# bcgsc/abyss

Measured on NVIDIA H100. Metric: k-mers/sec (Bloom insert + unitig extend), higher is better.
Workload: dtype u8

## Files before the change

abyss_b200/csrc/abb_api.cu:

```cuda
#include "abb_common.h"
#include "abb_insert.cuh"
#include "abb_shard.cuh"
#include <dlfcn.h>
#include <nccl.h>
#include <cub/device/device_scan.cuh>
#include <algorithm>
#include <cstdlib>
#include <cstring>
#include <new>
#include <vector>

namespace abb {

static thread_local char g_err[512] = "";

void set_error(const char* fmt, ...)
{
	va_list ap;
	va_start(ap, fmt);
	vsnprintf(g_err, sizeof g_err, fmt, ap);
	va_end(ap);
}

constexpr uint64_t kDefaultWindow = 1ULL << 17;
constexpr uint64_t kChunkSlots = 1ULL << 27;

static uint64_t next_pow2(uint64_t x)
{
	uint64_t p = 1;
	while (p < x)
		p <<= 1;
	return p;
}

int select_device(int device)
{
	int n = 0;
	cudaError_t e = cudaGetDeviceCount(&n);
	if (e != cudaSuccess || n <= 0) {
		set_error("no usable CUDA device (%s); libabyssb200 has no CPU fallback",
		          e == cudaSuccess ? "device count is 0" : cudaGetErrorString(e));
		return ABB_ENODEV;
	}
	if (device < 0 || device >= n) {
		set_error("device %d out of range (0..%d)", device, n - 1);
		return ABB_EINVAL;
	}
	ABB_CUDA(cudaSetDevice(device));
	return ABB_OK;
}

static FilterView view_of(const abb_filter* f)
{
	FilterView v;
	v.data = f->d_data.p;
	v.level_stride = f->level_stride();
	v.levels = f->levels;
	return v;
}

constexpr unsigned kMapLog2 = 25;
constexpr unsigned kShardMapLog2 = 27;

static uint64_t map_entries_for(uint64_t filter_size, unsigned lg)
{
	const uint64_t fit = std::max<uint64_t>(next_pow2(filter_size), 1024);
	return std::min<uint64_t>(1ULL << lg, fit);
}

static unsigned age_windows_for(uint64_t window)
{
	return (unsigned)std::min<uint64_t>(kMaxAgeWindows, ((1ULL << kPrioBits) - 2) / window - 1);
}

static int ensure_workspace(abb_filter* f, uint64_t window, unsigned lg)
{
	const uint64_t want_entries = map_entries_for(f->size, lg);
	if (f->d_carry.p && f->ws_window == window && f->ws_H == f->H && f->map_entries == want_entries)
		return ABB_OK;
	f->ws_window = 0;
	f->d_map[0] = f->d_map[1] = f->d_map[2] = nullptr;
	f->maps.reset();
	f->d_tags2[0].reset();
	f->d_tags2[1].reset();
	f->d_carry.reset();
	f->d_slotbits.reset();
	const size_t map_words = std::max<size_t>(want_entries / 4, 256) / sizeof(unsigned);
	f->tag_slots = next_pow2(8ULL * kCarryLanes * f->H);
	ABB_CHECK(f->maps.alloc(3 * map_words));
	ABB_CUDA(cudaMemsetAsync(f->maps.p, 0, 3 * map_words * sizeof(unsigned), f->stream));
	for (auto& tags : f->d_tags2) {
		ABB_CHECK(tags.alloc(f->tag_slots));
		ABB_CUDA(cudaMemsetAsync(tags.p, 0, f->tag_slots * sizeof(unsigned long long), f->stream));
	}
	ABB_CHECK(f->d_carry.alloc(3 * (window + kCarryLanes)));
	f->slotbit_words = ((uint64_t)age_windows_for(window) + 3) * window / 32 + 64;
	ABB_CHECK(f->d_slotbits.alloc(f->slotbit_words));
	ABB_CUDA(cudaMemsetAsync(f->d_slotbits.p, 0, f->slotbit_words * sizeof(unsigned), f->stream));
	for (int i = 0; i < 3; ++i)
		f->d_map[i] = f->maps.p + i * map_words;
	f->map_entries = want_entries;
	f->ws_window = window;
	f->ws_H = f->H;
	return ABB_OK;
}

#define ABB_DISPATCH_H(H, ...)            \
	do {                                  \
		if ((H) <= 4) {                   \
			constexpr int MAXH = 4;       \
			__VA_ARGS__;                  \
		} else if ((H) <= 8) {            \
			constexpr int MAXH = 8;       \
			__VA_ARGS__;                  \
		} else {                          \
			constexpr int MAXH = 32;      \
			__VA_ARGS__;                  \
		}                                 \
	} while (0)

static void set_l2_policy(abb_filter* f, bool on, int n_maps = 3)
{
	cudaStreamAttrValue attr;
	memset(&attr, 0, sizeof attr);
	if (on) {
		int max_persist = 0, max_window = 0;
		cudaDeviceGetAttribute(&max_persist, cudaDevAttrMaxPersistingL2CacheSize, f->device);
		cudaDeviceGetAttribute(&max_window, cudaDevAttrMaxAccessPolicyWindowSize, f->device);
		const size_t bytes = (size_t)n_maps * std::max<size_t>(f->map_entries / 4, 256);
		if (max_persist <= 0 || max_window <= 0)
			return;
		cudaDeviceSetLimit(cudaLimitPersistingL2CacheSize, std::min<size_t>(bytes, (size_t)max_persist));
		attr.accessPolicyWindow.base_ptr = f->d_map[0];
		attr.accessPolicyWindow.num_bytes = std::min<size_t>(bytes, (size_t)max_window);
		attr.accessPolicyWindow.hitRatio = std::min(1.0f, (float)max_persist / (float)bytes);
		attr.accessPolicyWindow.hitProp = cudaAccessPropertyPersisting;
		attr.accessPolicyWindow.missProp = cudaAccessPropertyStreaming;
	} else {
		attr.accessPolicyWindow.num_bytes = 0;
		attr.accessPolicyWindow.hitProp = cudaAccessPropertyNormal;
		attr.accessPolicyWindow.missProp = cudaAccessPropertyNormal;
	}
	cudaStreamSetAttribute(f->stream, cudaStreamAttributeAccessPolicyWindow, &attr);
	if (!on) {
		cudaCtxResetPersistingL2Cache();
		cudaDeviceSetLimit(cudaLimitPersistingL2CacheSize, 0);
	}
	cudaGetLastError();
}

struct PolicyHold {
	abb_filter* f;
	bool took;
	PolicyHold(abb_filter* f_, int n_maps) : f(f_), took(!f_->l2_policy_held && f_->d_map[0] != nullptr)
	{
		if (took) {
			set_l2_policy(f, true, n_maps);
			f->l2_policy_held = true;
		}
	}
	~PolicyHold()
	{
		if (took) {
			set_l2_policy(f, false);
			f->l2_policy_held = false;
		}
	}
	PolicyHold(const PolicyHold&) = delete;
	PolicyHold& operator=(const PolicyHold&) = delete;
};

template <int KIND, bool LITERAL, int MAXH>
static int launch_windows(const InsertArgs& args, int device, cudaStream_t st)
{
	static int grid_cache[64] = { 0 };
	int& grid = grid_cache[device & 63];
	if (grid == 0) {
		int per_sm = 0, sms = 0;
		ABB_CUDA(cudaOccupancyMaxActiveBlocksPerMultiprocessor(&per_sm, k_insert_windows<KIND, LITERAL, MAXH>, 256, 0));
		ABB_CUDA(cudaDeviceGetAttribute(&sms, cudaDevAttrMultiProcessorCount, device));
		grid = std::max(1, per_sm) * sms;
	}
	void* params[] = { (void*)&args };
	ABB_CUDA(cudaLaunchCooperativeKernel((void*)k_insert_windows<KIND, LITERAL, MAXH>, dim3((unsigned)grid), dim3(256), params, 0, st));
	return ABB_OK;
}

static int fold_profile(abb_filter* f)
{
	if (!f->profile || !f->prof_used)
		return ABB_OK;
	ABB_CUDA(cudaStreamSynchronize(f->stream));
	for (size_t i = 0; i + 1 < f->prof_used; i += 2) {
		float ms = 0;
		cudaEventElapsedTime(&ms, f->prof_ev[i], f->prof_ev[i + 1]);
		f->st.ms_commit += ms;
		f->st.commit_launches += 1;
	}
	f->st.commit_slots += f->prof_slots;
	f->prof_used = 0;
	f->prof_slots = 0;
	return ABB_OK;
}

template <bool LITERAL>
static int ordered_insert(abb_filter* f, const uint64_t* d_hashes, const uint8_t* d_valid, uint64_t n_slots)
{
	if (n_slots == 0)
		return ABB_OK;
	if (f->kind == ABB_BIT) {
		ABB_DISPATCH_H(f->H, (k_bits_insert<LITERAL, MAXH><<<blocks_for(n_slots, 256), 256, 0, f->stream>>>(
		                         d_hashes, d_valid, n_slots, f->cfg, f->d_data.p)));
		f->st.launches += 1;
		ABB_CUDA(cudaGetLastError());
		return ABB_OK;
	}
	ABB_CHECK(ensure_workspace(f, f->window, kMapLog2));
	cudaStream_t st = f->stream;
	const uint64_t W = f->window;
	const uint64_t n_windows = (n_slots + W - 1) / W;
	ABB_REQUIRE(n_windows < (1ULL << 31), "too many windows in one call");
	const uint64_t cap = W + kCarryLanes;
	InsertArgs a;
	a.hashes = d_hashes;
	a.valid = d_valid;
	a.n_slots = n_slots;
	a.window = (unsigned)W;
	a.w_begin = 0;
	a.n_windows = (unsigned)n_windows;
	a.cfg = f->cfg;
	for (int i = 0; i < 3; ++i) {
		a.map[i].w = f->d_map[i];
		a.map[i].mask = f->map_entries - 1;
	}
	for (int i = 0; i < 2; ++i) {
		a.tags[i] = f->d_tags2[i].p;
		a.carry[i] = f->d_carry.p + (uint64_t)i * cap;
	}
	a.tag_cap = (unsigned)f->tag_slots;
	a.f = view_of(f);
	a.age_off = (unsigned)(age_windows_for(W) * W);
	a.drain_age = a.age_off / 3 * 2;
	a.ctl = f->d_ctl.p;
	a.stats = f->d_stats.p;
	uint64_t* sorted = f->d_carry.p + 2 * cap;
	ABB_CUDA(cudaMemsetAsync(f->d_ctl.p, 0, sizeof(InsertCtl), st));
	ABB_CUDA(cudaMemsetAsync(f->d_map[0], 0, 3 * std::max<size_t>(f->map_entries / 4, 256), st));
	for (int i = 0; i < 2; ++i)
		ABB_CUDA(cudaMemsetAsync(f->d_tags2[i].p, 0, f->tag_slots * sizeof(unsigned long long), st));
	const bool counting = f->kind == ABB_COUNTING;
	PolicyHold policy(f, 3);
	while (a.w_begin < a.n_windows) {
		const bool timed = f->profile && f->prof_used + 2 <= f->prof_ev.size();
		if (timed)
			cudaEventRecord(f->prof_ev[f->prof_used++], st);
		ABB_DISPATCH_H(f->H, {
			if (counting)
				ABB_CHECK((launch_windows<0, LITERAL, MAXH>(a, f->device, st)));
			else
				ABB_CHECK((launch_windows<1, LITERAL, MAXH>(a, f->device, st)));
		});
		if (timed)
			cudaEventRecord(f->prof_ev[f->prof_used++], st);
		InsertCtl h;
		ABB_CUDA(cudaMemcpyAsync(&h, f->d_ctl.p, sizeof h, cudaMemcpyDeviceToHost, st));
		ABB_CUDA(cudaStreamSynchronize(st));
		ABB_REQUIRE(h.resume > a.w_begin && h.resume <= a.n_windows, "insert kernel made no progress (window %u of %u)", h.resume, a.n_windows);
		if (timed)
			f->prof_slots += std::min<uint64_t>(n_slots, (uint64_t)h.resume * W) - (uint64_t)a.w_begin * W;
		const int which = 1 - (int)((h.resume - 1) & 1);
		const uint64_t w0 = (uint64_t)(h.resume - 1) * W;
		const uint64_t lo_slot = w0 > (uint64_t)a.age_off + W ? w0 - a.age_off - W : 0;
		ABB_DISPATCH_H(f->H, {
			if (counting)
				k_drain<0, LITERAL, MAXH><<<1, kDrainThreads, 0, st>>>(d_hashes, f->cfg, a.f, a.carry[which], a.ctl, which, 0, 1, f->d_slotbits.p, lo_slot,
				                                                      sorted, f->d_stats.p);
			else
				k_drain<1, LITERAL, MAXH><<<1, kDrainThreads, 0, st>>>(d_hashes, f->cfg, a.f, a.carry[which], a.ctl, which, 0, 1, f->d_slotbits.p, lo_slot,
				                                                      sorted, f->d_stats.p);
		});
		f->st.launches += 2;
		f->st.windows += h.resume - a.w_begin;
		a.w_begin = h.resume;
	}
	ABB_CUDA(cudaGetLastError());
	return fold_profile(f);
}

__global__ void k_chunk_bounds(const uint64_t* __restrict__ slot_offs, uint64_t n_reads, uint64_t cap,
                               uint64_t* __restrict__ bounds, unsigned max_chunks, unsigned* __restrict__ n_chunks)
{
	uint64_t r = 0;
	unsigned c = 0;
	bounds[0] = 0;
	while (r < n_reads && c + 1 < max_chunks) {
		const uint64_t limit = slot_offs[r] + cap;
		uint64_t lo = r + 1, hi = n_reads;
		while (lo < hi) {
			uint64_t mid = lo + (hi - lo + 1) / 2;
			if (slot_offs[mid] <= limit)
				lo = mid;
			else
				hi = mid - 1;
		}
		r = lo;
		bounds[++c] = r;
	}
	if (r < n_reads)
		bounds[++c] = n_reads;
	*n_chunks = c;
}

__global__ void __launch_bounds__(256)
k_count_valid(const uint8_t* __restrict__ valid, uint64_t n, unsigned long long* __restrict__ out)
{
	unsigned long long c = 0;
	for (uint64_t i = (uint64_t)blockIdx.x * blockDim.x + threadIdx.x; i < n; i += (uint64_t)gridDim.x * blockDim.x)
// ... 186 lines not shown
		f->st.ms_insert += ms;
		f->st.slots += slots;
	}
	unsigned long long nk = 0;
	ABB_CUDA(cudaMemcpyAsync(&nk, f->d_stats.p + kStatInsertKmers, sizeof nk, cudaMemcpyDeviceToHost, f->stream));
	ABB_CUDA(cudaStreamSynchronize(f->stream));
	f->st.kmers += nk;
	if (n_kmers_out)
		*n_kmers_out = nk;
	return ABB_OK;
}

struct NcclApi {
	void* h = nullptr;
	ncclResult_t (*GetUniqueId)(ncclUniqueId*) = nullptr;
	ncclResult_t (*CommInitRank)(ncclComm_t*, int, ncclUniqueId, int) = nullptr;
	ncclResult_t (*CommDestroy)(ncclComm_t) = nullptr;
	ncclResult_t (*AllReduce)(const void*, void*, size_t, ncclDataType_t, ncclRedOp_t, ncclComm_t, cudaStream_t) = nullptr;
	ncclResult_t (*AllGather)(const void*, void*, size_t, ncclDataType_t, ncclComm_t, cudaStream_t) = nullptr;
	ncclResult_t (*Send)(const void*, size_t, ncclDataType_t, int, ncclComm_t, cudaStream_t) = nullptr;
	ncclResult_t (*Recv)(void*, size_t, ncclDataType_t, int, ncclComm_t, cudaStream_t) = nullptr;
	ncclResult_t (*GroupStart)() = nullptr;
	ncclResult_t (*GroupEnd)() = nullptr;
	const char* (*GetErrorString)(ncclResult_t) = nullptr;
};
static NcclApi g_nccl;

static int load_nccl()
{
	if (g_nccl.h)
		return ABB_OK;
	const char* names[] = { getenv("ABB_NCCL_LIB"), "libnccl.so.2", "libnccl.so" };
	void* h = nullptr;
	for (const char* n : names)
		if (n && *n && (h = dlopen(n, RTLD_NOW | RTLD_GLOBAL)))
			break;
	if (!h) {
		set_error("cannot load NCCL (libnccl.so.2): %s", dlerror());
		return ABB_ENODEV;
	}
#define ABB_NCCL_SYM(field, name)                                        \
	do {                                                                 \
		*(void**)(&g_nccl.field) = dlsym(h, name);                       \
		if (!g_nccl.field) {                                             \
			set_error("NCCL library lacks %s", name);                    \
			return ABB_ENODEV;                                           \
		}                                                                \
	} while (0)
	ABB_NCCL_SYM(GetUniqueId, "ncclGetUniqueId");
	ABB_NCCL_SYM(CommInitRank, "ncclCommInitRank");
	ABB_NCCL_SYM(CommDestroy, "ncclCommDestroy");
	ABB_NCCL_SYM(AllReduce, "ncclAllReduce");
	ABB_NCCL_SYM(AllGather, "ncclAllGather");
	ABB_NCCL_SYM(Send, "ncclSend");
	ABB_NCCL_SYM(Recv, "ncclRecv");
	ABB_NCCL_SYM(GroupStart, "ncclGroupStart");
	ABB_NCCL_SYM(GroupEnd, "ncclGroupEnd");
	ABB_NCCL_SYM(GetErrorString, "ncclGetErrorString");
#undef ABB_NCCL_SYM
	g_nccl.h = h;
	return ABB_OK;
}

#define ABB_NCCL(call)                                                                                   \
	do {                                                                                                 \
		ncclResult_t r__ = (call);                                                                       \
		if (r__ != ncclSuccess) {                                                                        \
			abb::set_error("%s:%d: %s failed: %s", __FILE__, __LINE__, #call, g_nccl.GetErrorString(r__)); \
			return ABB_ECUDA;                                                                            \
		}                                                                                                \
	} while (0)

}

struct abb_comm {
	ncclComm_t comm = nullptr;
	int rank = 0, world = 1, device = 0;
};

namespace abb {

static uint64_t shard_chunk(uint64_t size, unsigned world) { return ((size + world - 1) / world + 15) & ~15ULL; }

static uint64_t sharded_window(const abb_filter* f, unsigned world)
{
	const uint64_t w = 2 * f->window * world;
	return std::min<uint64_t>(std::max<uint64_t>(w, 32), 1ULL << 21);
}

static int sharded_ordered_insert(abb_filter* f, abb_comm* c, const uint64_t* d_h0, const uint8_t* d_valid, uint64_t n_slots)
{
	if (n_slots == 0)
		return ABB_OK;
	const uint64_t W = sharded_window(f, (unsigned)c->world);
	ABB_CHECK(ensure_workspace(f, W, kShardMapLog2));
	const unsigned max_lanes = (unsigned)std::min<uint64_t>((uint64_t)kCarryLanes * (unsigned)c->world, W / 2 + kCarryLanes);
	ABB_CHECK(f->sh_buf.reserve(2 * (W + (uint64_t)max_lanes) + 64));
	cudaStream_t st = f->stream;
	const uint64_t n_windows = (n_slots + W - 1) / W;
	const unsigned age_off = (unsigned)(age_windows_for(W) * W);
	const unsigned drain_age = age_off / 3 * 2;
	const uint64_t cap = 3 * (W + kCarryLanes) / 2;
	uint64_t* carry[2] = { f->d_carry.p, f->d_carry.p + cap };
	ShardCtl* ctl = f->d_shard_ctl.p;
	const size_t map_bytes = std::max<size_t>(f->map_entries / 4, 256);
	ConflictMap maps[2] = { { f->d_map[0], f->map_entries - 1 }, { f->d_map[1], f->map_entries - 1 } };
	const uint64_t chunk = shard_chunk(f->size, (unsigned)c->world);
	Shard sh;
	sh.lo = std::min<uint64_t>(f->size, (uint64_t)c->rank * chunk);
	sh.hi = std::min<uint64_t>(f->size, sh.lo + chunk);
	{
		ShardCtl init;
		init.n_pending = 0;
		init.n_out = 0;
		init.lo_pending = ~0ULL;
		ABB_CUDA(cudaMemcpyAsync(ctl, &init, sizeof init, cudaMemcpyHostToDevice, st));
	}
	ABB_CUDA(cudaMemsetAsync(f->d_map[0], 0, 3 * map_bytes, st));
	unsigned n_in = 0;
	uint64_t oldest = 0;
	int in = 0, p = 0;
	uint8_t* buf = f->sh_buf.p;
	auto step = [&](uint64_t w0, unsigned n, uint64_t w1, unsigned n_next) -> int {
		const unsigned lanes_c = std::min<unsigned>(n_in, max_lanes);
		uint64_t tslots = 4096;
		while (tslots < 8ULL * lanes_c * f->H / (unsigned)c->world + 4096 && tslots < f->tag_slots)
			tslots <<= 1;
		const TagTable tab = { f->d_tags2[0].p, std::min<uint64_t>(tslots, f->tag_slots) - 1 };
		if (lanes_c)
			ABB_CUDA(cudaMemsetAsync(tab.e, 0, (tab.mask + 1) * sizeof(unsigned long long), st));
		const unsigned lanes = lanes_c + n;
		const uint64_t lo_slot = w0 > (uint64_t)age_off + W ? w0 - age_off - W : 0;
		uint8_t* pm = buf;
		uint8_t* ok = buf + lanes;
		const bool timed = f->profile && n && (f->st.windows % f->prof_stride) == 0 && f->prof_used + 2 <= f->prof_ev.size();
		ABB_DISPATCH_H(f->H, {
			if (lanes_c)
				k_sh_mark_carry<false, MAXH><<<blocks_for(lanes_c, 256), 256, 0, st>>>(d_h0, carry[in], lanes_c, w0, f->cfg, tab, age_off, maps[p], sh);
			if (timed)
				cudaEventRecord(f->prof_ev[f->prof_used++], st);
			k_sh_gather<false, MAXH><<<blocks_for((uint64_t)lanes_c + std::max(n, n_next), 256), 256, 0, st>>>(
			    d_h0, d_valid, w0, n, w1, n_next, f->cfg, maps[p], maps[1 - p], tab, f->d_data.p, age_off, carry[in], lanes_c, sh, pm, ok);
		});
		if (lanes) {
			ABB_NCCL(g_nccl.AllReduce(buf, buf, 2 * (size_t)lanes, ncclUint8, ncclMin, c->comm, st));
			ABB_DISPATCH_H(f->H, (k_sh_apply<false, MAXH><<<blocks_for((uint64_t)n_in + n, 256), 256, 0, st>>>(
			                         d_h0, d_valid, w0, n, f->cfg, tab, f->d_data.p, carry[in], n_in, lanes_c, sh, pm, ok, f->d_slotbits.p, lo_slot, ctl,
			                         f->d_stats.p)));
			if (timed) {
				cudaEventRecord(f->prof_ev[f->prof_used++], st);
				f->prof_slots += n;
			}
			k_sh_compact<<<1, kDrainThreads, 0, st>>>(f->d_slotbits.p, lo_slot, w0 + std::max<uint64_t>(n, 1), carry[1 - in], ctl, &ctl->n_out);
			unsigned h_n = 0;
			ABB_CUDA(cudaMemcpyAsync(&h_n, &ctl->n_out, sizeof h_n, cudaMemcpyDeviceToHost, st));
			ABB_CUDA(cudaMemcpyAsync(&oldest, carry[1 - in], sizeof oldest, cudaMemcpyDeviceToHost, st));
			ABB_CUDA(cudaStreamSynchronize(st));
			n_in = h_n;
			in = 1 - in;
			f->st.launches += 4;
		} else {
			if (timed)
				f->prof_used--;
			f->st.launches += 1;
		}
		return ABB_OK;
	};
	auto drain = [&](uint64_t w0, unsigned until) -> int {
		while (n_in > until) {
			ABB_CHECK(step(w0, 0, w0, 0));
			f->sh_drains += 1;
		}
		return ABB_OK;
	};
	f->prof_stride = f->prof_ev.empty() ? 1 : std::max<uint64_t>(1, (2 * n_windows + f->prof_ev.size() - 1) / f->prof_ev.size());
	PolicyHold policy(f, 2);
	ABB_CHECK(step(0, 0, 0, (unsigned)std::min<uint64_t>(W, n_slots)));
	p = 1 - p;
// ... 4 lines not shown
		const unsigned n_next = w + 1 < n_windows ? (unsigned)std::min<uint64_t>(W, n_slots - w1) : 0u;
		if (n_in > max_lanes)
			ABB_CHECK(drain(w0, max_lanes / 2));
		if (n_in && w0 - oldest > drain_age)
			ABB_CHECK(drain(w0, 0));
		ABB_CHECK(step(w0, n, w1, n_next));
		ABB_CUDA(cudaMemsetAsync(maps[p].w, 0, map_bytes, st));
		p = 1 - p;
		f->st.windows += 1;
	}
	ABB_CHECK(drain(n_slots, 0));
	ABB_CUDA(cudaGetLastError());
	return fold_profile(f);
}

}

using namespace abb;

extern "C" {

int abb_version(void) { return ABB_VERSION; }
const char* abb_last_error(void) { return g_err; }

int abb_device_count(void)
{
	int n = 0;
	cudaError_t e = cudaGetDeviceCount(&n);
	if (e != cudaSuccess) {
		set_error("cudaGetDeviceCount: %s", cudaGetErrorString(e));
		return ABB_ENODEV;
	}
	return n;
}

static int alloc_filter(std::unique_ptr<abb_filter> f, abb_filter** out);

int abb_filter_create(abb_filter** out, int kind, uint64_t size, unsigned num_hashes, unsigned k, unsigned arg,
                      const char* mask, int device)
{
	ABB_REQUIRE(out != nullptr, "abb_filter_create: out is NULL");
	*out = nullptr;
	ABB_REQUIRE(kind != ABB_KONNECTOR, "Konnector filters are created with abb_konnector_create");
	ABB_REQUIRE(kind == ABB_COUNTING || kind == ABB_BIT || kind == ABB_CASCADING, "unknown filter kind %d", kind);
	ABB_REQUIRE(num_hashes >= 1 && num_hashes <= kMaxHashes, "number of hash functions must be in 1..%u (MAX_HASHES)", kMaxHashes);
	ABB_REQUIRE(k >= 1 && k <= kMaxK, "k-mer size must be in 1..%u (MAX_KMER)", kMaxK);
	if (kind == ABB_COUNTING) {
		if (size % 8)
			size += 8 - size % 8;
	} else {
		ABB_REQUIRE(size % 8 == 0, "ERROR: Filter Size \"%llu\" is not a multiple of 8.", (unsigned long long)size);
	}
	ABB_REQUIRE(size >= 8, "filter size must be at least 8");
	ABB_REQUIRE(size < (1ULL << kPosBits), "filter size %llu exceeds the supported maximum 2^%u", (unsigned long long)size, kPosBits);
	unsigned levels = 1;
	if (kind == ABB_CASCADING) {
		ABB_REQUIRE(arg >= 1 && arg <= 255, "cascading filter needs 1..255 levels");
		levels = arg;
	}
	std::string m = mask ? mask : "";
	if (!m.empty()) {
		ABB_REQUIRE(m.size() == k, "spaced seed must be exactly k=%u characters long", k);
		for (char c : m)
			ABB_REQUIRE(c == '0' || c == '1', "spaced seed must contain only '0' and '1'");
		if (m.find('0') == std::string::npos)
			m.clear();
	}
	ABB_CHECK(select_device(device));

	std::unique_ptr<abb_filter> f(new (std::nothrow) abb_filter());
	if (!f) {
		set_error("out of host memory");
		return ABB_ENOMEM;
	}
	f->device = device;
	f->kind = kind;
	f->size = size;
	f->bytes_per_level = kind == ABB_COUNTING ? size : size / 8;
	f->H = num_hashes;
	f->k = k;
	f->threshold = kind == ABB_COUNTING ? arg : 0;
	f->levels = levels;
	f->mask = m;
	f->window = kDefaultWindow;
	f->cfg.H = num_hashes;
	f->cfg.k = k;
	f->cfg.mod = make_fastmod(size);
	for (unsigned i = 0; i < kMaxHashes; ++i)
		f->cfg.mult[i] = (uint64_t)i ^ ((uint64_t)k * kMultiSeed);
	return alloc_filter(std::move(f), out);
}

static int alloc_filter(std::unique_ptr<abb_filter> f, abb_filter** out)
{
	const unsigned k = f->k, levels = f->levels;
	ABB_CUDA(cudaStreamCreateWithFlags(f->stream.out(), cudaStreamNonBlocking));
	ABB_CUDA(cudaEventCreate(f->ev0.out()));
	ABB_CUDA(cudaEventCreate(f->ev1.out()));
	ABB_CHECK(f->d_data.alloc(f->level_stride() * levels + 4096));
	ABB_CUDA(cudaMemsetAsync(f->d_data.p, 0, f->level_stride() * levels, f->stream));
	ABB_CHECK(f->d_ctl.alloc(1));
	ABB_CUDA(cudaMemsetAsync(f->d_ctl.p, 0, sizeof(InsertCtl), f->stream));
	ABB_CHECK(f->d_shard_ctl.alloc(1));
	ABB_CHECK(f->d_stats.alloc(kStatWords));
	ABB_CUDA(cudaMemsetAsync(f->d_stats.p, 0, kStatWords * sizeof(unsigned long long), f->stream));
	if (!f->mask.empty()) {
		std::vector<uint8_t> care(k);
		for (unsigned i = 0; i < k; ++i)
			care[i] = f->mask[i] == '1';
		ABB_CHECK(f->d_care.alloc(k));
		ABB_CUDA(cudaMemcpyAsync(f->d_care.p, care.data(), k, cudaMemcpyHostToDevice, f->stream));
	}
	ABB_CUDA(cudaStreamSynchronize(f->stream));
	return hand_over(f, out);
}

int abb_konnector_create(abb_filter** out, uint64_t full_bits, unsigned k, unsigned levels, uint64_t hash_seed, uint64_t start_bit,
                         uint64_t end_bit, int device)
{
	ABB_REQUIRE(out != nullptr, "abb_konnector_create: out is NULL");
	*out = nullptr;
	ABB_REQUIRE(k >= 1 && k <= kMaxK, "k-mer size must be in 1..%u (MAX_KMER)", kMaxK);
	ABB_REQUIRE(full_bits >= 2, "a Konnector filter needs at least 2 bits");
	ABB_REQUIRE(start_bit <= end_bit && end_bit < full_bits, "window [%llu, %llu] is not inside a filter of %llu bits",
	            (unsigned long long)start_bit, (unsigned long long)end_bit, (unsigned long long)full_bits);
	ABB_REQUIRE(levels >= 1 && levels <= 255, "a Konnector filter needs 1..255 levels");
	ABB_CHECK(select_device(device));
	std::unique_ptr<abb_filter> f(new (std::nothrow) abb_filter());
	if (!f) {
		set_error("out of host memory");
		return ABB_ENOMEM;
	}
	f->device = device;
	f->kind = ABB_KONNECTOR;
	f->size = end_bit - start_bit + 1;
	f->bytes_per_level = (f->size + 7) / 8;
	f->H = 1;
	f->k = k;
	f->levels = levels;
	f->kon_full = full_bits;
	f->kon_start = start_bit;
	f->kon_seed = hash_seed;
	return alloc_filter(std::move(f), out);
}

int abb_filter_destroy(abb_filter* f)
{
	if (!f)
		return ABB_OK;
	cudaSetDevice(f->device);
	cudaStreamSynchronize(f->stream);
	if (f->copy_stream)
		cudaStreamSynchronize(f->copy_stream);
	delete f;
	return ABB_OK;
}

unsigned abb_filter_kmer_size(const abb_filter* f) { return f ? f->k : 0; }
unsigned abb_filter_hash_num(const abb_filter* f) { return f ? f->H : 0; }
uint64_t abb_filter_size(const abb_filter* f) { return f ? f->size : 0; }
uint64_t abb_filter_size_in_bytes(const abb_filter* f) { return f ? f->bytes_per_level : 0; }
unsigned abb_filter_threshold(const abb_filter* f) { return f ? f->threshold : 0; }
unsigned abb_filter_levels(const abb_filter* f) { return f ? f->levels : 0; }

int abb_filter_set_threshold(abb_filter* f, unsigned threshold)
{
	ABB_REQUIRE(f, "NULL filter");
	if (f->kind != ABB_COUNTING) {
		set_error("threshold only applies to counting filters");
		return ABB_ESTATE;
	}
	f->threshold = threshold;
	return ABB_OK;
}

int abb_filter_set_profiling(abb_filter* f, int on)
{
	ABB_REQUIRE(f, "NULL filter");
	ABB_CUDA(cudaSetDevice(f->device));
	f->profile = on != 0;
	if (f->profile && f->prof_ev.empty()) {
		std::vector<Event> ev(2048);
		for (auto& e : ev)
			ABB_CUDA(cudaEventCreate(e.out()));
		f->prof_ev = std::move(ev);
	}
	return ABB_OK;
}

int abb_filter_set_window(abb_filter* f, uint64_t window_slots)
{
	ABB_REQUIRE(f, "NULL filter");
	if (window_slots == 0)
		window_slots = kDefaultWindow;
	ABB_REQUIRE(window_slots >= 32 && window_slots <= (1ULL << 20) - 64, "window must be in [32, 2^20 - 64]");
	ABB_CUDA(cudaSetDevice(f->device));
	ABB_CUDA(cudaStreamSynchronize(f->stream));
	f->window = window_slots;
	return ABB_OK;
}

int abb_insert_reads_dev(abb_filter* f, const char* d_bases, const uint64_t* d_offsets, uint64_t n_reads,
                         uint64_t n_bases, uint64_t* n_kmers_out)
{
	(void)n_bases;
	ABB_REQUIRE(f, "NULL filter");
	ABB_REQUIRE(n_reads == 0 || (d_bases && d_offsets), "NULL read buffers");
	ABB_CUDA(cudaSetDevice(f->device));
	if (f->kind == ABB_KONNECTOR)
		return kon_insert_reads_dev(f, (const uint8_t*)d_bases, d_offsets, n_reads, n_kmers_out);
	return insert_reads_dev(f, (const uint8_t*)d_bases, d_offsets, n_reads, n_kmers_out);
}

int abb_insert_reads(abb_filter* f, const char* bases, const uint64_t* offsets, uint64_t n_reads, uint64_t* n_kmers_out)
{
	ABB_REQUIRE(f, "NULL filter");
	if (n_kmers_out)
		*n_kmers_out = 0;
	if (n_reads == 0)
		return ABB_OK;
	ABB_CHECK(check_read_batch(bases, offsets, n_reads));
	const uint64_t n_bases = offsets[n_reads];
	ABB_CUDA(cudaSetDevice(f->device));
	constexpr uint64_t kPiece = 256ULL << 20;
	const bool in_pieces = f->kind != ABB_KONNECTOR && n_bases > kPiece;
	ABB_CHECK(stage_read_batch(in_pieces ? nullptr : bases, offsets, n_reads, f->bases, f->offs, f->stream));
	f->resident_reads = n_reads;
	if (f->kind == ABB_KONNECTOR)
		return kon_insert_reads_dev(f, f->bases.p, f->offs.p, n_reads, n_kmers_out);
	if (!in_pieces)
		return insert_reads_dev(f, f->bases.p, f->offs.p, n_reads, n_kmers_out);
	if (!f->copy_stream)
		ABB_CUDA(cudaStreamCreateWithFlags(f->copy_stream.out(), cudaStreamNonBlocking));
	if (f->kind != ABB_BIT)
		ABB_CHECK(ensure_workspace(f, f->window, kMapLog2));
	PolicyHold policy(f, 3);
	PendingCopy pc;
	pc.h_offs = offsets;
	pc.piece = kPiece;
	pc.n_pieces = (size_t)((n_bases + kPiece - 1) / kPiece);
	while (f->copy_ev.size() < pc.n_pieces) {
		Event ev;
		ABB_CUDA(cudaEventCreateWithFlags(ev.out(), cudaEventDisableTiming));
		f->copy_ev.push_back(std::move(ev));
	}
	ABB_CUDA(cudaEventRecord(f->ev0, f->stream));
	ABB_CUDA(cudaStreamWaitEvent(f->copy_stream, f->ev0, 0));
	for (size_t i = 0; i < pc.n_pieces; ++i) {
		const uint64_t b0 = (uint64_t)i * kPiece, b1 = std::min<uint64_t>(n_bases, b0 + kPiece);
		ABB_CUDA(cudaMemcpyAsync(f->bases.p + b0, bases + b0, b1 - b0, cudaMemcpyHostToDevice, f->copy_stream));
		ABB_CUDA(cudaEventRecord(f->copy_ev[i], f->copy_stream));
	}
	const int rc = insert_reads_dev(f, f->bases.p, f->offs.p, n_reads, n_kmers_out, nullptr, &pc);
	ABB_CUDA(cudaStreamSynchronize(f->copy_stream));
	return rc;
}

static bool shard_policy(int world)
{
	static int min_world = -1;
	if (min_world < 0) {
		const char* e = getenv("ABB_SHARD_MIN_WORLD");
		min_world = e ? std::max(2, atoi(e)) : 4;
	}
	return world > 1 && world >= min_world;
}

int abb_insert_reads_sharded(abb_filter* f, abb_comm* c, const char* bases, const uint64_t* offsets, uint64_t n_reads, int finalize,
                             uint64_t* n_kmers_out)
{
	ABB_REQUIRE(f && c, "NULL argument");
	ABB_REQUIRE_NTHASH(f);
	if (!shard_policy(c->world)) {
		ABB_REQUIRE(f->kind == ABB_COUNTING, "the sharded insert is implemented for counting filters");
		ABB_REQUIRE(f->device == c->device, "filter and communicator live on different devices");
		f->replicated_insert = true;
		(void)finalize;
		return abb_insert_reads(f, bases, offsets, n_reads, n_kmers_out);
	}
	if (n_kmers_out)
		*n_kmers_out = 0;
	ABB_CHECK(check_read_batch(bases, offsets, n_reads));
	ABB_CUDA(cudaSetDevice(f->device));
	ABB_CHECK(stage_read_batch(bases, offsets, n_reads, f->bases, f->offs, f->stream));
	f->resident_reads = n_reads;
	return abb_insert_reads_sharded_dev(f, c, (const char*)f->bases.p, f->offs.p, n_reads, finalize, n_kmers_out);
}

int abb_filter_resident_reads(abb_filter* f, const char** d_bases, const uint64_t** d_offsets, uint64_t* n_reads)
{
	ABB_REQUIRE(f && d_bases && d_offsets && n_reads, "NULL argument");
	*d_bases = (const char*)f->bases.p;
	*d_offsets = f->offs.p;
	*n_reads = f->resident_reads;
	return ABB_OK;
}

int abb_insert_hashes(abb_filter* f, const uint64_t* hashes, uint64_t n)
{
	ABB_REQUIRE(f, "NULL filter");
	ABB_REQUIRE_NTHASH(f);
	if (n == 0)
		return ABB_OK;
	ABB_REQUIRE(hashes, "NULL hashes");
	ABB_CUDA(cudaSetDevice(f->device));
	ABB_CHECK(f->lit.reserve(n * f->H));
	ABB_CUDA(cudaMemcpyAsync(f->lit.p, hashes, n * f->H * sizeof(uint64_t), cudaMemcpyHostToDevice, f->stream));
	ABB_CHECK(ordered_insert<true>(f, f->lit.p, nullptr, n));
	ABB_CUDA(cudaStreamSynchronize(f->stream));
	f->st.kmers += n;
	return ABB_OK;
}

int abb_hash_reads_dev(abb_filter* f, const char* d_bases, const uint64_t* d_offsets, uint64_t n_reads, uint64_t* d_h0,
                       uint8_t* d_valid, uint64_t capacity, uint64_t* n_slots_out)
{
	ABB_REQUIRE(f, "NULL filter");
	ABB_REQUIRE_NTHASH(f);
// ... 457 lines not shown
```

abyss_b200/csrc/abb_insert.cuh:

```cuda
#pragma once
#include "abb_common.h"
#include "abb_device.cuh"
#include "abb_graph.cuh"
#include <cooperative_groups.h>
#include <cuda/barrier>
#include <cuda_runtime.h>

namespace abb {
namespace cg = cooperative_groups;

constexpr unsigned kPrioBits = 28;
constexpr unsigned kMaxAgeWindows = 48;
constexpr unsigned kCarryLanes = 1u << 16;
constexpr unsigned kPosBits = 36;
constexpr uint64_t kPrioMask = (1ULL << kPrioBits) - 1;

struct TagTable {
	unsigned long long* e;
	uint64_t mask;
};

ABB_D uint64_t tag_pack(uint64_t pos, uint64_t prio) { return ((pos + 1) << kPrioBits) | prio; }
ABB_D uint64_t tag_home(uint64_t pos, const TagTable& t)
{
// ... 246 lines not shown
static __global__ void __launch_bounds__(kHashWarps * 32)
k_hash_segments(const uint8_t* __restrict__ bases, const uint64_t* __restrict__ seg_beg, const unsigned* __restrict__ seg_len,
                const uint64_t* __restrict__ seg_slot, uint64_t n_segs, unsigned k, uint64_t* __restrict__ h0_out,
                uint8_t* __restrict__ valid_out)
{
	__shared__ uint64_t sP[kHashWarps][kRing];
	__shared__ uint64_t sQ[kHashWarps][kRing];
	__shared__ unsigned sB[kHashWarps][kRing];
	const int warp = threadIdx.x >> 5, lane = threadIdx.x & 31;
	for (uint64_t r = (uint64_t)blockIdx.x * kHashWarps + warp; r < n_segs; r += (uint64_t)gridDim.x * kHashWarps) {
		const unsigned L = seg_len[r];
		if (L < k)
			continue;
		hash_one_read(bases, seg_beg[r], L, seg_slot[r], k, sP[warp], sQ[warp], sB[warp], lane, h0_out, valid_out);
	}
}

static __global__ void __launch_bounds__(kHashWarps * 32)
k_hash_reads_masked(const uint8_t* __restrict__ bases, const uint64_t* __restrict__ offs,
                    const uint64_t* __restrict__ slot_offs, uint64_t slot_base, uint64_t n_reads, unsigned k,
                    const uint8_t* __restrict__ care, uint64_t* __restrict__ h0_out, uint8_t* __restrict__ valid_out)
{
	const int warp = threadIdx.x >> 5, lane = threadIdx.x & 31;
	for (uint64_t r = (uint64_t)blockIdx.x * kHashWarps + warp; r < n_reads; r += (uint64_t)gridDim.x * kHashWarps) {
		const uint64_t beg = offs[r];
		const unsigned L = (unsigned)(offs[r + 1] - beg);
		if (L < k)
			continue;
		hash_one_read_masked(bases, beg, L, slot_offs[r] - slot_base, k, care, lane, h0_out, valid_out);
	}
}

static __global__ void __launch_bounds__(kHashWarps * 32)
k_hash_segments_masked(const uint8_t* __restrict__ bases, const uint64_t* __restrict__ seg_beg,
                       const unsigned* __restrict__ seg_len, const uint64_t* __restrict__ seg_slot, uint64_t n_segs, unsigned k,
                       const uint8_t* __restrict__ care, uint64_t* __restrict__ h0_out, uint8_t* __restrict__ valid_out)
{
	const int warp = threadIdx.x >> 5, lane = threadIdx.x & 31;
	for (uint64_t r = (uint64_t)blockIdx.x * kHashWarps + warp; r < n_segs; r += (uint64_t)gridDim.x * kHashWarps) {
		const unsigned L = seg_len[r];
		if (L < k)
			continue;
		hash_one_read_masked(bases, seg_beg[r], L, seg_slot[r], k, care, lane, h0_out, valid_out);
	}
}

static __global__ void k_window_counts(const uint64_t* __restrict__ offs, uint64_t n_reads, unsigned k,
                                uint64_t* __restrict__ counts)
{
	uint64_t r = (uint64_t)blockIdx.x * blockDim.x + threadIdx.x;
	if (r < n_reads) {
		uint64_t L = offs[r + 1] - offs[r];
		counts[r] = L >= k ? L - k + 1 : 0;
	}
}


template <bool LITERAL, int MAXH>
ABB_D void slot_positions(const uint64_t* __restrict__ hashes, uint64_t s, const HashCfg& cfg, uint64_t* pos)
{
	if (LITERAL) {
#pragma unroll
		for (int i = 0; i < MAXH; ++i)
			if (i < (int)cfg.H)
				pos[i] = fastmod_u64(hashes[s * cfg.H + i], cfg.mod);
	} else {
		const uint64_t h0 = hashes[s];
#pragma unroll
		for (int i = 0; i < MAXH; ++i)
			if (i < (int)cfg.H)
				pos[i] = nth_pos(h0, cfg, i);
	}
}
template <bool LITERAL>
ABB_D uint64_t slot_position(const uint64_t* __restrict__ hashes, uint64_t s, const HashCfg& cfg, unsigned i)
{
	return LITERAL ? fastmod_u64(hashes[s * cfg.H + i], cfg.mod) : nth_pos(hashes[s], cfg, i);
}

struct ConflictMap {
	unsigned* w;
	uint64_t mask;
};
ABB_D void map_mark(const ConflictMap& m, uint64_t pos)
{
	const uint64_t e = pos & m.mask;
	const unsigned sh = (unsigned)(e & 15) * 2;
	const unsigned old = atomicOr(&m.w[e >> 4], 1u << sh);
	if (((old >> sh) & 3u) == 1u)
		atomicOr(&m.w[e >> 4], 2u << sh);
}
template <int MAXH>
ABB_D void map_mark_all(const ConflictMap& m, const uint64_t* pos, unsigned H)
{
	unsigned old[MAXH];
#pragma unroll
	for (int i = 0; i < MAXH; ++i)
		if (i < (int)H) {
			const uint64_t e = pos[i] & m.mask;
			old[i] = atomicOr(&m.w[e >> 4], 1u << ((unsigned)(e & 15) * 2));
		}
#pragma unroll
	for (int i = 0; i < MAXH; ++i)
		if (i < (int)H) {
			const uint64_t e = pos[i] & m.mask;
			const unsigned sh = (unsigned)(e & 15) * 2;
			if (((old[i] >> sh) & 3u) == 1u)
				atomicOr(&m.w[e >> 4], 2u << sh);
		}
}
ABB_D void map_mark_carried(const ConflictMap& m, uint64_t pos)
{
	const uint64_t e = pos & m.mask;
	atomicOr(&m.w[e >> 4], 3u << ((unsigned)(e & 15) * 2));
}
ABB_D unsigned map_get(const ConflictMap& m, uint64_t pos)
{
	const uint64_t e = pos & m.mask;
	return (__ldcg(&m.w[e >> 4]) >> ((unsigned)(e & 15) * 2)) & 3u;
}

template <int KIND, int MAXH>
ABB_D void apply_alone(const FilterView& f, const uint64_t* pos, const unsigned* v, unsigned H)
{
	if (KIND == 0) {
		unsigned mn = 255;
#pragma unroll
		for (int i = 0; i < MAXH; ++i)
			if (i < (int)H)
				mn = min(mn, v[i]);
		if (mn == 255)
			return;
#pragma unroll
		for (int i = 0; i < MAXH; ++i)
			if (i < (int)H && v[i] == mn)
				__stcg(f.data + pos[i], (uint8_t)(mn + 1));
	} else
		apply_cascading(f, pos, H);
}

struct InsertArgs {
	const uint64_t* hashes;
	const uint8_t* valid;
	uint64_t n_slots;
	unsigned window;
	unsigned w_begin, n_windows;
	HashCfg cfg;
	ConflictMap map[3];
	unsigned long long* tags[2];
	unsigned tag_cap;
	FilterView f;
	unsigned age_off, drain_age;
	uint64_t* carry[2];
	InsertCtl* ctl;
	unsigned long long* stats;
};

ABB_D unsigned tag_mask_for(unsigned n_carried, unsigned H, unsigned cap)
{
	unsigned want = 4096;
	while (want < 8u * n_carried * H && want < cap)
		want <<= 1;
	return min(want, cap) - 1;
}

template <int KIND, bool LITERAL, int MAXH>
__global__ void __launch_bounds__(256, 4)
k_insert_windows(const InsertArgs a)
{
	cg::grid_group grid = cg::this_grid();
	const uint64_t T = (uint64_t)gridDim.x * blockDim.x;
	const uint64_t gtid = (uint64_t)blockIdx.x * blockDim.x + threadIdx.x;
	const unsigned H = a.cfg.H;
	const uint64_t W = a.window;
	uint64_t pos[MAXH];
	unsigned v[MAXH];
	if (a.w_begin == 0) {
		const unsigned n0 = (unsigned)min((uint64_t)W, a.n_slots);
		for (uint64_t t = gtid; t < n0; t += T)
			if (!a.valid || a.valid[t]) {
				slot_positions<LITERAL, MAXH>(a.hashes, t, a.cfg, pos);
				map_mark_all<MAXH>(a.map[0], pos, H);
			}
		grid.sync();
	}
	for (unsigned w = a.w_begin; w < a.n_windows; ++w) {
		const int in = (int)(w & 1), out = 1 - in;
		const ConflictMap& mcur = a.map[w % 3];
		const ConflictMap& mnext = a.map[(w + 1) % 3];
		const ConflictMap& mold = a.map[(w + 2) % 3];
		const uint64_t w0 = (uint64_t)w * W, w1 = w0 + W;
		const unsigned n = (unsigned)min(W, a.n_slots - w0);
		const unsigned n_next = w + 1 < a.n_windows ? (unsigned)min(W, a.n_slots - w1) : 0u;
		const unsigned n_in = a.ctl->n_carry[in];
		const TagTable tcur = { a.tags[in], a.ctl->tag_mask[in] };
		const unsigned old_mask_out = a.ctl->tag_mask[out];
		for (uint64_t id = gtid; id < (uint64_t)n_in + max(n, n_next); id += T) {
			if (id < n_in) {
				const uint64_t s = a.carry[in][id];
				const uint64_t prio = s + a.age_off - w0;
				slot_positions<LITERAL, MAXH>(a.hashes, s, a.cfg, pos);
				if (KIND == 0) {
#pragma unroll
					for (int i = 0; i < MAXH; ++i)
						if (i < (int)H)
							v[i] = __ldcg(a.f.data + pos[i]);
				}
				bool owner = true;
				uint64_t where[MAXH];
#pragma unroll
				for (int i = 0; i < MAXH; ++i)
					if (i < (int)H)
						owner &= tag_owner_at(tcur, pos[i], &where[i]) == prio;
				if (owner) {
					apply_alone<KIND, MAXH>(a.f, pos, v, H);
#pragma unroll
					for (int i = 0; i < MAXH; ++i)
						if (i < (int)H)
							tag_release_at(tcur, pos[i], where[i]);
				} else {
					a.carry[out][atomicAdd(&a.ctl->n_carry[out], 1u)] = s;
					if (w0 - s > a.drain_age)
						a.ctl->old_flag = 1;
				}
				continue;
			}
			const uint64_t t = id - n_in;
			const bool do_apply = t < n && (!a.valid || a.valid[w0 + t]);
			const bool do_mark = t < n_next && (!a.valid || a.valid[w1 + t]);
			uint64_t pos2[MAXH];
			if (do_apply)
				slot_positions<LITERAL, MAXH>(a.hashes, w0 + t, a.cfg, pos);
			if (do_mark)
				slot_positions<LITERAL, MAXH>(a.hashes, w1 + t, a.cfg, pos2);
			unsigned again = 0;
			if (do_apply) {
#pragma unroll
				for (int i = 0; i < MAXH; ++i)
					if (i < (int)H)
						again |= map_get(mcur, pos[i]);
				if (KIND == 0) {
#pragma unroll
					for (int i = 0; i < MAXH; ++i)
						if (i < (int)H)
							v[i] = __ldcg(a.f.data + pos[i]);
				}
			}
			if (do_mark)
				map_mark_all<MAXH>(mnext, pos2, H);
			if (do_apply) {
				if (!(again & 2u))
					apply_alone<KIND, MAXH>(a.f, pos, v, H);
				else {
					a.carry[out][atomicAdd(&a.ctl->n_carry[out], 1u)] = w0 + t;
					atomicAdd(&a.stats[kStatDeferred], 1ULL);
				}
			}
		}
		for (uint64_t i = gtid; i <= old_mask_out; i += T)
			a.tags[out][i] = 0;
		uint4* mw = reinterpret_cast<uint4*>(mold.w);
		const uint64_t words4 = (mold.mask + 1) / 64;
		for (uint64_t i = gtid; i < words4; i += T)
			mw[i] = make_uint4(0, 0, 0, 0);
		grid.sync();
		const unsigned n_out = a.ctl->n_carry[out];
		const bool stop = n_out > kCarryLanes || a.ctl->old_flag != 0;
		const bool last = w + 1 == a.n_windows;
		const unsigned new_mask = tag_mask_for(n_out, H, a.tag_cap);
		if (!stop && !last) {
			const TagTable tnext = { a.tags[out], new_mask };
			for (uint64_t i = gtid; i < n_out; i += T) {
				const uint64_t s = a.carry[out][i];
				slot_positions<LITERAL, MAXH>(a.hashes, s, a.cfg, pos);
				const uint64_t prio = s + a.age_off - w1;
#pragma unroll
				for (int j = 0; j < MAXH; ++j)
					if (j < (int)H) {
						tag_reserve(tnext, pos[j], prio);
						map_mark_carried(mnext, pos[j]);
					}
			}
		}
		if (gtid == 0) {
			a.ctl->n_carry[in] = 0;
			a.ctl->tag_mask[out] = (!stop && !last) ? new_mask : 0u;
			a.ctl->resume = w + 1;
		}
		grid.sync();
		if (stop)
			return;
	}
}

constexpr unsigned kDrainThreads = 1024;
constexpr unsigned kDrainPos = 2048;
constexpr unsigned kDrainMap = 4096;

ABB_D unsigned block_exclusive_scan(unsigned x, unsigned* warp_sums , unsigned* total)
{
	const unsigned lane = threadIdx.x & 31, warp = threadIdx.x >> 5;
	unsigned incl = x;
#pragma unroll
	for (int d = 1; d < 32; d <<= 1) {
		unsigned y = __shfl_up_sync(0xffffffffu, incl, d);
		if (lane >= (unsigned)d)
			incl += y;
	}
	if (lane == 31)
		warp_sums[warp] = incl;
	__syncthreads();
	if (warp == 0) {
		unsigned wsum = warp_sums[lane];
		unsigned winc = wsum;
#pragma unroll
		for (int d = 1; d < 32; d <<= 1) {
			unsigned y = __shfl_up_sync(0xffffffffu, winc, d);
			if (lane >= (unsigned)d)
				winc += y;
		}
		warp_sums[lane] = winc - wsum;
		if (lane == 31)
			*total = winc;
	}
	__syncthreads();
	return warp_sums[warp] + incl - x;
}

ABB_D unsigned enumerate_presence(unsigned* __restrict__ bw, unsigned words, uint64_t first_slot, uint64_t* __restrict__ out,
                                  unsigned* warp_sums, unsigned* total)
{
	const unsigned per = (words + blockDim.x - 1) / blockDim.x;
	const unsigned wb = min(words, threadIdx.x * per), we = min(words, wb + per);
	unsigned cnt = 0;
	for (unsigned wd = wb; wd < we; ++wd)
		cnt += __popc(__ldcg(&bw[wd]));
	unsigned at = block_exclusive_scan(cnt, warp_sums, total);
	for (unsigned wd = wb; wd < we; ++wd) {
		unsigned m = __ldcg(&bw[wd]);
		if (m)
			bw[wd] = 0;
		while (m) {
			const unsigned b = __ffs(m) - 1;
			m &= m - 1;
			out[at++] = first_slot + (uint64_t)wd * 32 + b;
		}
	}
// ... 270 lines not shown
```

Before: 646.5 million.

## Split conflict map into two hashed halves and double default insert window

Replaces the single 2-bit conflict map with two half-size maps indexed by the masked position and a multiplicative hash of it. A slot counts as conflicting only if both halves agree, which cuts false conflicts caused by aliasing. With fewer false conflicts, the default window for large filters doubles to 2^18, giving fewer grid syncs per k-mer. The cost is twice the atomics per mark, and the larger window raises carry and tag pressure.

```diff
diff --git a/abyss_b200/csrc/abb_api.cu b/abyss_b200/csrc/abb_api.cu
--- a/abyss_b200/csrc/abb_api.cu
+++ b/abyss_b200/csrc/abb_api.cu
@@ -22,7 +22,6 @@
 	va_end(ap);
 }
 
-constexpr uint64_t kDefaultWindow = 1ULL << 17;
 constexpr uint64_t kChunkSlots = 1ULL << 27;
 
 static uint64_t next_pow2(uint64_t x)
@@ -60,12 +59,19 @@
 }
 
 constexpr unsigned kMapLog2 = 25;
+static_assert(kMapLog2 - 1 <= kMapHalfLog2Max, "half B of a conflict map cannot index more than 2^24 entries");
+constexpr uint64_t kDefaultWindow = 1ULL << 18;
+constexpr uint64_t kExactMapWindow = 1ULL << 17;
+static uint64_t default_window(uint64_t filter_size)
+{
+	return filter_size > (1ULL << (kMapLog2 - 1)) ? kDefaultWindow : kExactMapWindow;
+}
 constexpr unsigned kShardMapLog2 = 27;
 
-static uint64_t map_entries_for(uint64_t filter_size, unsigned lg)
+static uint64_t map_entries_for(uint64_t filter_size, unsigned lg, unsigned halves)
 {
 	const uint64_t fit = std::max<uint64_t>(next_pow2(filter_size), 1024);
-	return std::min<uint64_t>(1ULL << lg, fit);
+	return halves * std::min<uint64_t>((1ULL << lg) / halves, fit);
 }
 
 static unsigned age_windows_for(uint64_t window)
@@ -73,9 +79,9 @@
 	return (unsigned)std::min<uint64_t>(kMaxAgeWindows, ((1ULL << kPrioBits) - 2) / window - 1);
 }
 
-static int ensure_workspace(abb_filter* f, uint64_t window, unsigned lg)
-{
-	const uint64_t want_entries = map_entries_for(f->size, lg);
+static int ensure_workspace(abb_filter* f, uint64_t window, unsigned lg, unsigned halves)
+{
+	const uint64_t want_entries = map_entries_for(f->size, lg, halves);
 	if (f->d_carry.p && f->ws_window == window && f->ws_H == f->H && f->map_entries == want_entries)
 		return ABB_OK;
 	f->ws_window = 0;
@@ -215,7 +221,7 @@
 		ABB_CUDA(cudaGetLastError());
 		return ABB_OK;
 	}
-	ABB_CHECK(ensure_workspace(f, f->window, kMapLog2));
+	ABB_CHECK(ensure_workspace(f, f->window, kMapLog2, 2));
 	cudaStream_t st = f->stream;
 	const uint64_t W = f->window;
 	const uint64_t n_windows = (n_slots + W - 1) / W;
@@ -229,10 +235,8 @@
 	a.w_begin = 0;
 	a.n_windows = (unsigned)n_windows;
 	a.cfg = f->cfg;
-	for (int i = 0; i < 3; ++i) {
-		a.map[i].w = f->d_map[i];
-		a.map[i].mask = f->map_entries - 1;
-	}
+	for (int i = 0; i < 3; ++i)
+		a.map[i].a = { f->d_map[i], f->map_entries / 2 - 1 };
 	for (int i = 0; i < 2; ++i) {
 		a.tags[i] = f->d_tags2[i].p;
 		a.carry[i] = f->d_carry.p + (uint64_t)i * cap;
@@ -585,10 +589,11 @@
 
 static uint64_t shard_chunk(uint64_t size, unsigned world) { return ((size + world - 1) / world + 15) & ~15ULL; }
 
+constexpr uint64_t kShardRankWindow = 1ULL << 18;
 static uint64_t sharded_window(const abb_filter* f, unsigned world)
 {
-	const uint64_t w = 2 * f->window * world;
-	return std::min<uint64_t>(std::max<uint64_t>(w, 32), 1ULL << 21);
+	const uint64_t per_rank = f->window == default_window(f->size) ? kShardRankWindow : 2 * f->window;
+	return std::min<uint64_t>(std::max<uint64_t>(per_rank * world, 32), 1ULL << 21);
 }
 
 static int sharded_ordered_insert(abb_filter* f, abb_comm* c, const uint64_t* d_h0, const uint8_t* d_valid, uint64_t n_slots)
@@ -596,7 +601,7 @@
 	if (n_slots == 0)
 		return ABB_OK;
 	const uint64_t W = sharded_window(f, (unsigned)c->world);
-	ABB_CHECK(ensure_workspace(f, W, kShardMapLog2));
+	ABB_CHECK(ensure_workspace(f, W, kShardMapLog2, 1));
 	const unsigned max_lanes = (unsigned)std::min<uint64_t>((uint64_t)kCarryLanes * (unsigned)c->world, W / 2 + kCarryLanes);
 	ABB_CHECK(f->sh_buf.reserve(2 * (W + (uint64_t)max_lanes) + 64));
 	cudaStream_t st = f->stream;
@@ -767,7 +772,7 @@
 	f->threshold = kind == ABB_COUNTING ? arg : 0;
 	f->levels = levels;
 	f->mask = m;
-	f->window = kDefaultWindow;
+	f->window = default_window(size);
 	f->cfg.H = num_hashes;
 	f->cfg.k = k;
 	f->cfg.mod = make_fastmod(size);
@@ -877,7 +882,7 @@
 {
 	ABB_REQUIRE(f, "NULL filter");
 	if (window_slots == 0)
-		window_slots = kDefaultWindow;
+		window_slots = default_window(f->size);
 	ABB_REQUIRE(window_slots >= 32 && window_slots <= (1ULL << 20) - 64, "window must be in [32, 2^20 - 64]");
 	ABB_CUDA(cudaSetDevice(f->device));
 	ABB_CUDA(cudaStreamSynchronize(f->stream));
@@ -918,7 +923,7 @@
 	if (!f->copy_stream)
 		ABB_CUDA(cudaStreamCreateWithFlags(f->copy_stream.out(), cudaStreamNonBlocking));
 	if (f->kind != ABB_BIT)
-		ABB_CHECK(ensure_workspace(f, f->window, kMapLog2));
+		ABB_CHECK(ensure_workspace(f, f->window, kMapLog2, 2));
 	PolicyHold policy(f, 3);
 	PendingCopy pc;
 	pc.h_offs = offsets;
diff --git a/abyss_b200/csrc/abb_insert.cuh b/abyss_b200/csrc/abb_insert.cuh
--- a/abyss_b200/csrc/abb_insert.cuh
+++ b/abyss_b200/csrc/abb_insert.cuh
@@ -352,42 +352,72 @@
 	unsigned* w;
 	uint64_t mask;
 };
-ABB_D void map_mark(const ConflictMap& m, uint64_t pos)
-{
-	const uint64_t e = pos & m.mask;
+ABB_D unsigned map_touch(const ConflictMap& m, uint64_t key)
+{
+	const uint64_t e = key & m.mask;
+	return atomicOr(&m.w[e >> 4], 1u << ((unsigned)(e & 15) * 2));
+}
+ABB_D void map_touch_again(const ConflictMap& m, uint64_t key, unsigned old)
+{
+	const uint64_t e = key & m.mask;
 	const unsigned sh = (unsigned)(e & 15) * 2;
-	const unsigned old = atomicOr(&m.w[e >> 4], 1u << sh);
 	if (((old >> sh) & 3u) == 1u)
 		atomicOr(&m.w[e >> 4], 2u << sh);
 }
+ABB_D void map_mark_carried(const ConflictMap& m, uint64_t key)
+{
+	const uint64_t e = key & m.mask;
+	atomicOr(&m.w[e >> 4], 3u << ((unsigned)(e & 15) * 2));
+}
+ABB_D unsigned map_get(const ConflictMap& m, uint64_t key)
+{
+	const uint64_t e = key & m.mask;
+	return (__ldcg(&m.w[e >> 4]) >> ((unsigned)(e & 15) * 2)) & 3u;
+}
+ABB_D void map_clear(const ConflictMap& m, uint64_t gtid, uint64_t T)
+{
+	uint4* mw = reinterpret_cast<uint4*>(m.w);
+	const uint64_t words4 = (m.mask + 1) / 64;
+	for (uint64_t i = gtid; i < words4; i += T)
+		mw[i] = make_uint4(0, 0, 0, 0);
+}
+
+struct ConflictMap2 {
+	ConflictMap a;
+	ABB_D ConflictMap b() const { return { a.w + (a.mask + 1) / 16, a.mask }; }
+};
+constexpr unsigned kMapHalfLog2Max = 24;
+ABB_D uint64_t map_key_b(uint64_t pos) { return (pos * 0xD6E8FEB86659FD93ULL) >> (64 - kMapHalfLog2Max); }
 template <int MAXH>
-ABB_D void map_mark_all(const ConflictMap& m, const uint64_t* pos, unsigned H)
-{
-	unsigned old[MAXH];
+ABB_D void map_mark_all(const ConflictMap2& m, const uint64_t* pos, unsigned H)
+{
+	unsigned old_a[MAXH], old_b[MAXH];
 #pragma unroll
 	for (int i = 0; i < MAXH; ++i)
 		if (i < (int)H) {
-			const uint64_t e = pos[i] & m.mask;
-			old[i] = atomicOr(&m.w[e >> 4], 1u << ((unsigned)(e & 15) * 2));
+			old_a[i] = map_touch(m.a, pos[i]);
+			old_b[i] = map_touch(m.b(), map_key_b(pos[i]));
 		}
 #pragma unroll
 	for (int i = 0; i < MAXH; ++i)
 		if (i < (int)H) {
-			const uint64_t e = pos[i] & m.mask;
-			const unsigned sh = (unsigned)(e & 15) * 2;
-			if (((old[i] >> sh) & 3u) == 1u)
-				atomicOr(&m.w[e >> 4], 2u << sh);
-		}
-}
-ABB_D void map_mark_carried(const ConflictMap& m, uint64_t pos)
-{
-	const uint64_t e = pos & m.mask;
-	atomicOr(&m.w[e >> 4], 3u << ((unsigned)(e & 15) * 2));
-}
-ABB_D unsigned map_get(const ConflictMap& m, uint64_t pos)
-{
-	const uint64_t e = pos & m.mask;
-	return (__ldcg(&m.w[e >> 4]) >> ((unsigned)(e & 15) * 2)) & 3u;
+			map_touch_again(m.a, pos[i], old_a[i]);
+			map_touch_again(m.b(), map_key_b(pos[i]), old_b[i]);
+		}
+}
+ABB_D void map_mark_carried(const ConflictMap2& m, uint64_t pos)
+{
+	map_mark_carried(m.a, pos);
+	map_mark_carried(m.b(), map_key_b(pos));
+}
+ABB_D unsigned map_get(const ConflictMap2& m, uint64_t pos)
+{
+	return map_get(m.a, pos) & map_get(m.b(), map_key_b(pos));
+}
+ABB_D void map_clear(const ConflictMap2& m, uint64_t gtid, uint64_t T)
+{
+	map_clear(m.a, gtid, T);
+	map_clear(m.b(), gtid, T);
 }
 
 template <int KIND, int MAXH>
@@ -416,7 +446,7 @@
 	unsigned window;
 	unsigned w_begin, n_windows;
 	HashCfg cfg;
-	ConflictMap map[3];
+	ConflictMap2 map[3];
 	unsigned long long* tags[2];
 	unsigned tag_cap;
 	FilterView f;
@@ -456,9 +486,9 @@
 	}
 	for (unsigned w = a.w_begin; w < a.n_windows; ++w) {
 		const int in = (int)(w & 1), out = 1 - in;
-		const ConflictMap& mcur = a.map[w % 3];
-		const ConflictMap& mnext = a.map[(w + 1) % 3];
-		const ConflictMap& mold = a.map[(w + 2) % 3];
+		const ConflictMap2& mcur = a.map[w % 3];
+		const ConflictMap2& mnext = a.map[(w + 1) % 3];
+		const ConflictMap2& mold = a.map[(w + 2) % 3];
 		const uint64_t w0 = (uint64_t)w * W, w1 = w0 + W;
 		const unsigned n = (unsigned)min(W, a.n_slots - w0);
 		const unsigned n_next = w + 1 < a.n_windows ? (unsigned)min(W, a.n_slots - w1) : 0u;
@@ -529,10 +559,7 @@
 		}
 		for (uint64_t i = gtid; i <= old_mask_out; i += T)
 			a.tags[out][i] = 0;
-		uint4* mw = reinterpret_cast<uint4*>(mold.w);
-		const uint64_t words4 = (mold.mask + 1) / 64;
-		for (uint64_t i = gtid; i < words4; i += T)
-			mw[i] = make_uint4(0, 0, 0, 0);
+		map_clear(mold, gtid, T);
 		grid.sync();
 		const unsigned n_out = a.ctl->n_carry[out];
 		const bool stop = n_out > kCarryLanes || a.ctl->old_flag != 0;
```

Result: faster. 726.1 million, median of 6 (+12.3%).
